# joeylitalien/drmlt-mitsuba

Measured on AMD Instinct MI355X. Metric: mutations/sec (accepted+rejected), higher is better.
Workload: dtype f32

## Files before the change

drmlt-mitsuba_amd/csrc/device_path.h:

```cpp
#pragma once
#include "device_bsdf.h"
#include "device_math.h"
#include "device_sampler.h"
#include "device_types.h"

struct Hit {
    int prim;
    float t, u, v;
};

typedef uint32_t u32x4_t __attribute__((ext_vector_type(4)));
template <class T> DEV T load_global16(const T *p) {
    static_assert(sizeof(T) % 16 == 0, "records are read in 16-byte words");
    typedef const u32x4_t __attribute__((address_space(1))) *GQ;
    const GQ q = (GQ) (uintptr_t) p;
    union { T v; u32x4_t w[sizeof(T) / 16]; } u;
#pragma unroll
    for (unsigned i = 0; i < sizeof(T) / 16u; ++i) u.w[i] = q[i];
    return u.v;
}
DEV f3 smooth_record_sum(const DParams &P, float index_bits, float u, float v) {
    typedef float f32x3_t __attribute__((ext_vector_type(3)));
    typedef const char __attribute__((address_space(1))) *GB;
    typedef const f32x3_t __attribute__((address_space(1))) *GQ;
// ... 422 lines not shown
        load(p, A);
        for (int i = 0; i < n; i += 2, p += 2) {
            PINF(A);
            load(p + 1, B);
            test_flat<TRI>(A, o, d, tmin, best_t, best_uv, best_ks);
            if (i + 1 < n) {
                PINF(B);
                load(p + 2, A);
                test_flat<TRI>(B, o, d, tmin, best_t, best_uv, best_ks);
            }
        }
    }
#undef PINF
    Hit h{-1, best_t, best_uv.x, best_uv.y};
    if (best_ks >= 0) {
        if (best_ks & BOX_FACE_FLAG) {
            const uint32_t hc = (uint32_t) best_ks & 0xffffu;
            const float uu = (hc & 2u) ? h.v : h.u, vv = (hc & 2u) ? h.u : h.v;
            h.u = (hc & 4u) ? 1.f - uu : uu;
            h.v = (hc & 8u) ? 1.f - vv : vv;
            best_ks = (int) (((hc >> 4) & 3u) | ((hc >> 6) << 8));
        }
        h.prim = best_ks >> 8;
        if ((best_ks & 0xff) == PRIM_QUAD2) {
            const bool second = h.v > h.u;
            const float uu = second ? h.u : h.u - h.v, vv = second ? h.v - h.u : h.v;
            h.prim += second ? 1 : 0;
            h.u = uu; h.v = vv;
        }
    }
    return h;
}

template <int FEAT = 15> DEV Hit trace(const DParams &P, f3 o, f3 d, float tmin, float tmax, bool any_hit) {
    if ((FEAT & 8) && P.use_bvh) return trace_bvh(P, o, d, tmin, tmax, any_hit);
    if (P.prims_flat) {
        Hit h = P.has_plain_tri ? trace_flat<true>(P, o, d, tmin, tmax) : trace_flat<false>(P, o, d, tmin, tmax);
        if (FEAT & 4)
            for (int i = P.n_flat; i < P.n_prims; ++i) {
                ScalarPrimPtr sp = (ScalarPrimPtr) (uintptr_t) P.prims;
                DPrim G;
#pragma unroll
                for (int k = 0; k < 12; ++k) G.m[k] = sp[i].m[k];
                const int ks = sp[i].kind_shade;
                G.type = PRIM_SPHERE; G.shade = ks >> 8;
                intersect_prim<4>(G, G.shade, o, d, tmin, h);
            }
        return h;
    }
    return trace_brute<FEAT>(P, o, d, tmin, tmax);
}

struct GlobalTables {
    const DShade *sh; const DBsdf *bs; const DEmitter *em;
    DEV DShade shade(int i) const { return load_global16(sh + i); }
    DEV DBsdf bsdf(int i) const { return load_global16(bs + i); }
    DEV DEmitter emitter(int i) const { return load_global16(em + i); }
    DEV float emitter_cdf_lo(int i) const { return load_global_f32(&em[i].cdf_lo); }
    DEV DShade emitter_shade(int, const DEmitter &E) const { return shade(E.prim); }
};
struct LdsTables {
    uint32_t shade_off, bsdf_off, emit_off;
    DEV DShade shade(int i) const {
        const float4 *q = reinterpret_cast<const float4 *>(&lds_x[shade_off + (uint32_t) i * 16u]);
        const float4 a = q[0], b = q[1], c = q[2], d = q[3];
        DShade s;
// ... 622 lines not shown
```

drmlt-mitsuba_amd/csrc/drmlt_capi.cpp:

```cpp
#include "../../include/drmlt_abi.h"
#include "device_types.h"
#include "drmlt_ctx.h"
#include "scene_prep.h"
#include "bdpt_layers.h"

#include <hip/hip_runtime.h>

#include <algorithm>
#include <chrono>
#include <cmath>
#include <cstdarg>
#include <cstdio>
#include <cstdlib>
#include <cstring>
#include <string>
#include <vector>

void launch_bootstrap(const DParams &P, uint32_t n, float *lum_out, hipStream_t st);
void launch_init_chains(const DParams &P, const uint32_t *seed_index, const float *seed_lum, hipStream_t st);
void launch_mutate(const ChainPlan &plan, const DParams &P, uint32_t n_mut, uint32_t mut_base, hipStream_t st);
void launch_eval_paths(const DParams &P, const float *u, uint32_t n, uint32_t dim, float *out8, hipStream_t st);
void launch_bootstrap_mmlt(const DParams &P, uint32_t n, float *lum_out, size_t lds, hipStream_t st);
void launch_init_chains_mmlt(const DParams &P, const uint32_t *seed_index, const float *seed_lum, size_t lds, hipStream_t st);
void launch_mutate_mmlt(const ChainPlan &plan, const DParams &P, uint32_t n_mut, uint32_t mut_base, hipStream_t st);
// ... 583 lines not shown
    }
    launch_develop(ctx->P.film, d_direct.as<float>(), ctx->P.importance, (float) factor, n, d_out.as<float>(), ctx->stream);
    HIP_TRY(ctx, hipGetLastError());
    HIP_TRY(ctx, hipMemcpyAsync(out_rgb, d_out.p, (size_t) n * sizeof(float), hipMemcpyDeviceToHost, ctx->stream));
    HIP_TRY(ctx, hipStreamSynchronize(ctx->stream));
    return DRMLT_OK;
}

int drmlt_stats_get(drmlt_ctx *ctx, drmlt_stats *o) {
    if (!ctx || !o) return DRMLT_E_INVALID;
    HIP_TRY(ctx, hipSetDevice(ctx->device));
    unsigned long long v[32];
    HIP_TRY(ctx, hipMemcpyAsync(v, ctx->d_stats.p, sizeof v, hipMemcpyDeviceToHost, ctx->stream));
    HIP_TRY(ctx, hipStreamSynchronize(ctx->stream));
    if ((ctx->P.debug & 128) && ctx->cfg.technique == DRMLT_TECH_BDPT)
        fprintf(stderr, "[drmlt stamps] bdpt cycles per wave, summed: walks %llu pair loop %llu whole chain loop %llu | evaluations %llu | stages (all evaluations) %llu, weights + splats %llu, counters + commit %llu\n",
                v[16], v[17], v[18], v[19], v[20], v[21], v[22]);
    else if ((ctx->P.debug & 128) && ctx->P.kernel_variant == 5)
        fprintf(stderr, "[drmlt v5] cycles per wave, summed: bookkeeping %llu step %llu trace %llu | outer iterations %llu, bookkeeping branches %llu (%.1f chains each), "
                        "stepping chains per iteration %.1f, trace phases %llu starting with %.1f lanes, refills %llu\n",
                v[16], v[18], v[17], v[19], v[23], v[23] ? (double) v[24] / v[23] : 0.0, v[19] ? (double) v[25] / v[19] : 0.0, v[20], v[20] ? (double) v[21] / v[20] : 0.0, v[22]);
    else if (ctx->P.debug & 128)
        fprintf(stderr, "[drmlt stamps] cycles: mh %llu trace %llu step %llu | iterations %llu mh-branches %llu tracing-lanes %llu\n",
                v[16], v[17], v[18], v[19], v[20], v[21]),
        fprintf(stderr, "[drmlt stamps] mh sections: decide+splat %llu commit %llu start %llu fill %llu\n", v[22], v[23], v[24], v[25]),
        fprintf(stderr, "[drmlt stamps] iterations by chains tracing (of 32): 0: %llu, 1-4: %llu, 5-8: %llu, 9-16: %llu, 17-24: %llu, 25-32: %llu\n", v[26], v[27], v[28], v[29], v[30], v[31]);
    if (ctx->knobs.verbose && v[12])
        fprintf(stderr, "[drmlt bvh] wave iterations: inner %llu (%.1f lanes each), leaf %llu (%.1f lanes each)\n", v[12], (double) v[10] / (double) v[12], v[13],
                v[13] ? (double) v[11] / (double) v[13] : 0.0);
    if (ctx->knobs.verbose && ctx->P.kernel_variant == 4)
        fprintf(stderr, "[drmlt v4] waves through the orbital rule body: %llu\n", v[14]),
        fprintf(stderr, "[drmlt v4] waves through a one-light build: %llu\n", v[15]);
    if (ctx->knobs.verbose && ctx->P.kernel_variant == 4 && !(ctx->P.debug & 128))
        fprintf(stderr, "[drmlt v4] waves through k_mutate_w2: %llu\n", v[16]);
    if ((ctx->P.debug & 1024) && v[20] && ctx->P.kernel_variant != 5)
        fprintf(stderr, "[drmlt bvh] lanes at slice start, of 64: tracing %.1f, chain waiting for its partner %.1f, chain parked for bookkeeping %.1f, helper idle %.1f, flush %.1f (%llu slices)\n",
                (double) v[21] / v[20], (double) v[22] / v[20], (double) v[23] / v[20], (double) v[24] / v[20], (double) v[25] / v[20], v[20]);
    memset(o, 0, sizeof *o);
    const uint64_t M = ctx->mutations;
    const uint64_t n_large = v[0], acc1_l = v[1], acc1_b = v[2], sec_l = v[3], sec_b = v[4], acc2_l = v[5], acc2_b = v[6], n_rev = v[7];
    if (ctx->cfg.algo == DRMLT_ALGO_PSSMLT) {
        o->overall_base = M;               o->overall_acc = acc1_l + acc1_b;
        o->large_base = n_large;           o->large_acc = acc1_l;
        o->bold_base = M - n_large;        o->bold_acc = acc1_b;
    } else if (!ctx->cfg.use_mixture) {
        o->first_base = M;                 o->first_acc = acc1_l + acc1_b;
        o->large_base = n_large;           o->large_acc = acc1_l;
        o->bold_base = M - n_large;        o->bold_acc = acc1_b;
        o->second_base = sec_l + sec_b;    o->second_acc = acc2_l + acc2_b;
        o->second_large_base = sec_l;      o->second_large_acc = acc2_l;
        o->second_bold_base = sec_b;       o->second_bold_acc = acc2_b;
        o->overall_base = M + sec_l + sec_b;
        o->overall_acc = acc1_l + acc1_b + acc2_l + acc2_b;
    } else {
        o->second_base = sec_b;            o->second_acc = acc2_b;
        o->first_base = M - sec_b;         o->first_acc = acc1_l + acc1_b;
        o->large_base = n_large;           o->large_acc = acc1_l;
        o->bold_base = M - n_large - sec_b; o->bold_acc = acc1_b;
        o->overall_base = M;               o->overall_acc = acc1_l + acc1_b + acc2_b;
    }
    o->mutations = M;
    o->path_evals = M + sec_l + sec_b + n_rev;
    o->rays = v[8];
    o->accepted = acc1_l + acc1_b + acc2_l + acc2_b;
    o->kernel_ms = ctx->kernel_ms;
    o->seed_ms = ctx->seed_ms;
    o->n_chains = ctx->n_chains;
// ... 243 lines not shown
```

drmlt-mitsuba_amd/csrc/kernels.hip:

```cpp
#include <algorithm>
#include <cstdlib>
#include <cstdio>
#include <type_traits>
#include "device_path.h"

#include "kernel_common.h"
#include "launch_plan.h"

__device__ __attribute__((noinline)) DSplat eval_boot_sample(const DParams &P, uint32_t index, uint32_t &nd) {
    Sampler smp;
    smp.key0 = P.key0; smp.key1 = P.key1; smp.chain = P.boot_stream; smp.major = index;
    smp.mode = SM_BOOT; smp.arr = nullptr;
    uint32_t nr;
    return eval_path(P, smp, nr, nd);
}

__global__ void __launch_bounds__(64) k_bootstrap(DParams P, uint32_t n, float *lum_out) {
    uint32_t i = blockIdx.x * blockDim.x + threadIdx.x;
    if (i >= n) return;
    uint32_t nd;
    DSplat s = eval_boot_sample(P, i, nd);
    lum_out[i] = s.lum;
    if (P.boot_weighted) { normalize_splat(s, P); lum_out[(size_t) n + i] = s.lum; }
}
// ... 1058 lines not shown
        helper_has_ray = lower_keeps_u(0u, sr.valid ? 1u : 0u) != 0u;
#else
        const float ox = from_lower(sr.o.x), oy = from_lower(sr.o.y), oz = from_lower(sr.o.z);
        const float dx = from_lower(sr.d.x), dy = from_lower(sr.d.y), dz = from_lower(sr.d.z);
        const float t0 = from_lower(sr.tmin), t1 = from_lower(sr.tmax);
        const float vf = from_lower(sr.valid ? 1.f : 0.f);
        if (helper) {
            ps.o = mk3(ox, oy, oz); ps.d = mk3(dx, dy, dz); ps.tmin = t0; ps.tmax = t1;
            helper_has_ray = vf != 0.f;
        }
#endif
    }
    SECTION_PARAMS(Pe);
    const V4Layout<RULE_ORBITAL> Y = v4_layout<RULE_ORBITAL>(Pe, V4_QCAP);
    if (qn + 32u > Y.L.qcap) W2_FLUSH(Pe, Y.L, qn, lane);
    v4_enqueue(Y.L, qn, live && cum > 0.f, cs.cur.px, cs.cur.py, cs.cur.r * cum, cs.cur.g * cum, cs.cur.b * cum);
    W2_FLUSH(Pe, Y.L, qn, lane);
    if (live) {
        RowSampler smp = Y.smp;
        smp.set_roles(roles, Y.group, sub);
        for (uint32_t k = 0; k < Y.D; ++k) Pe.x[(size_t) k * Pe.n_chains + c] = smp.x(k);
        Pe.cur_lum[c] = cs.cur.lum; Pe.cur_px[c] = cs.cur.px; Pe.cur_py[c] = cs.cur.py;
        Pe.cur_r[c] = cs.cur.r; Pe.cur_g[c] = cs.cur.g; Pe.cur_b[c] = cs.cur.b;
        if (Pe.chain_done) Pe.chain_done[c] = base + cs.it;
    }
    if (Pe.chain_done && !reported && lane == 0) atomicSub(Pe.waves_left, 1u);
    flush_counters(Pe, ct, lane);
    const unsigned long long decided = wave_sum((live && !helper) ? cs.it : 0u);
    if (lane == 0) atomicAdd(Pe.stats + 9, decided);
}
#undef W2_SECTION
#undef W2_FLUSH

#define V5_STACK32_CAP 25
#ifndef V5_ROWS_MEM_WAVES
#define V5_ROWS_MEM_WAVES 3
#endif
#ifndef V5_ROWS_MEM_STACK32_CAP
#define V5_ROWS_MEM_STACK32_CAP 25
#endif
enum { RS_IDLE = 0, RS_BUSY = 1, RS_DONE = 2 };

struct V5Lds {
    uint32_t coin_off, list_off;
    uint32_t q_off;
    uint32_t pool_off;
    uint32_t ring_off;
    uint32_t status_off;
};
DEV V5Lds v5_layout(uint32_t D, uint32_t qcap, bool coin_rows) {
    V5Lds L;
    L.coin_off = D * 64u;
    L.list_off = L.coin_off + (coin_rows ? 4u * 64u : 0u);
    L.q_off = L.list_off + 64u;
    L.pool_off = L.q_off + 5u * qcap;
    L.ring_off = L.pool_off + 8u * V5_SLOTS;
    L.status_off = L.ring_off + V5_SLOTS / 4u;
    return L;
}

template <int FEAT, bool STACK16, bool OVF, bool STAMPS = false, bool LDS_TABLES = false, bool ROWS_MEM = false>
__global__ void __launch_bounds__(CHAIN_BLOCK, ROWS_MEM ? V5_ROWS_MEM_WAVES : 2) k_mutate_v5(DParams P, uint32_t n_mut, uint32_t mut_base) {
    constexpr bool FLAT = (FEAT & 8) == 0;
    typedef typename std::conditional<ROWS_MEM, RowsMem, RowsLds>::type RowsT;
    typedef PoolRowSampler<RowsT> SamplerT;
    constexpr uint32_t QCAP = (FLAT || STACK16) ? V5_QCAP : V5_QCAP_STACK32;
// ... 483 lines not shown
    for (size_t i = (size_t) blockIdx.x * blockDim.x + threadIdx.x; i < n; i += (size_t) gridDim.x * blockDim.x) dst[i] += src[i];
}
void launch_accumulate(float *dst, const float *src, size_t n, hipStream_t st) {
    hipLaunchKernelGGL(k_accumulate, dim3((unsigned) std::min<size_t>((n + 255) / 256, AUX_GRID_CAP)), dim3(256), 0, st, dst, src, n);
}

void launch_bootstrap(const DParams &P, uint32_t n, float *lum_out, hipStream_t st) {
    hipLaunchKernelGGL(k_bootstrap, dim3((n + 63) / 64), dim3(64), 0, st, P, n, lum_out);
}
void launch_init_chains(const DParams &P, const uint32_t *seed_index, const float *seed_lum, hipStream_t st) {
    hipLaunchKernelGGL(k_init_chains, dim3((P.n_chains + 63) / 64), dim3(64), 0, st, P, seed_index, seed_lum);
}
void launch_mutate(const ChainPlan &plan, const DParams &P, uint32_t n_mut, uint32_t mut_base, hipStream_t st) {
    if (plan.verbose && !plan.note.empty()) fprintf(stderr, "%s\n", plan.note.c_str());
#define LAUNCH(...) hipLaunchKernelGGL((__VA_ARGS__), dim3(plan.grid), dim3(CHAIN_BLOCK), plan.lds, st, P, n_mut, mut_base); break
#define LAUNCH_RULE(FEAT, ...) if (orbital) { LAUNCH(k_mutate_v4<FEAT | V4_ORBITAL_BUILD, __VA_ARGS__>); } LAUNCH(k_mutate_v4<FEAT, __VA_ARGS__>)
#define LAUNCH_LIGHT(...) if (one_light) { LAUNCH_RULE(V4_ONE_LIGHT_BUILD, __VA_ARGS__); } LAUNCH_RULE(0, __VA_ARGS__)
    const bool orbital = rule_is_orbital(P), one_light = scene_has_one_light(P);
    switch (plan.build) {
    case Build::PSSMLT: LAUNCH(k_mutate_pssmlt);
    case Build::V5_F0_ROWS: LAUNCH(k_mutate_v5<0, true, false, false, true, true>);   case Build::V5_F1_ROWS: LAUNCH(k_mutate_v5<1, true, false, false, true, true>);
    case Build::V5_F3_ROWS: LAUNCH(k_mutate_v5<3, true, false, false, true, true>);   case Build::V5_F7_ROWS: LAUNCH(k_mutate_v5<7, true, false, false, true, true>);
    case Build::V5_F7_GLOBAL: LAUNCH(k_mutate_v5<7, true, false, false, false>);      case Build::V5_F0_STAMPS: LAUNCH(k_mutate_v5<0, true, false, true, true>);
    case Build::V5_F0: LAUNCH(k_mutate_v5<0, true, false, false, true>);             case Build::V5_F1: LAUNCH(k_mutate_v5<1, true, false, false, true>);
    case Build::V5_F3: LAUNCH(k_mutate_v5<3, true, false, false, true>);             case Build::V5_F7: LAUNCH(k_mutate_v5<7, true, false, false, true>);
    case Build::V5_F8_S32_ROWS: LAUNCH(k_mutate_v5<8, false, true, false, false, true>); case Build::V5_F15_S32_ROWS: LAUNCH(k_mutate_v5<15, false, true, false, false, true>);
    case Build::V5_F8_OVF_ROWS: LAUNCH(k_mutate_v5<8, true, true, false, false, true>);  case Build::V5_F15_OVF_ROWS: LAUNCH(k_mutate_v5<15, true, true, false, false, true>);
    case Build::V5_F8_ROWS: LAUNCH(k_mutate_v5<8, true, false, false, false, true>);     case Build::V5_F15_ROWS: LAUNCH(k_mutate_v5<15, true, false, false, false, true>);
    case Build::V5_F8_S32: LAUNCH(k_mutate_v5<8, false, true>); case Build::V5_F15_S32: LAUNCH(k_mutate_v5<15, false, true>);
    case Build::V5_F8_OVF: LAUNCH(k_mutate_v5<8, true, true>);  case Build::V5_F15_OVF: LAUNCH(k_mutate_v5<15, true, true>);
    case Build::V5_F8_STAMPS: LAUNCH(k_mutate_v5<8, true, false, true>); case Build::V5_F8: LAUNCH(k_mutate_v5<8, true, false>); case Build::V5_F15: LAUNCH(k_mutate_v5<15, true, false>);
    case Build::V4_F0_STAMPS: LAUNCH_LIGHT(true, true);
    case Build::V4_F0:
        if (plan.w2 && orbital && one_light) { LAUNCH(k_mutate_w2); }
        LAUNCH_LIGHT(true, false);
    case Build::V4_F3_STAMPS: LAUNCH(k_mutate_v4<3, true, true>); case Build::V4_F3: LAUNCH_RULE(3, true, false); case Build::V4_F7: LAUNCH_RULE(7, true, false);
    case Build::V4_F15_S32: LAUNCH(k_mutate_v4<15, true, false, false, true>); case Build::V4_F15_OVF: LAUNCH(k_mutate_v4<15, true, false, true, true>);
    case Build::V4_F15: LAUNCH(k_mutate_v4<15, true, false, true>);            case Build::V4_F7_GLOBAL: LAUNCH(k_mutate_v4<7, false, false>);
    case Build::V4_F8_S32_GLOBAL: LAUNCH(k_mutate_v4<8, false, false, false, true>); case Build::V4_F15_S32_GLOBAL: LAUNCH(k_mutate_v4<15, false, false, false, true>);
    case Build::V4_F15_OVF_GLOBAL: LAUNCH(k_mutate_v4<15, false, false, true, true>); case Build::V4_F15_STAMPS_GLOBAL: LAUNCH(k_mutate_v4<15, false, true, true>);
    case Build::V4_F8_GLOBAL: LAUNCH(k_mutate_v4<8, false, false, true>);            case Build::V4_F15_GLOBAL: LAUNCH(k_mutate_v4<15, false, false, true>);
    case Build::V3_F0: LAUNCH(k_mutate_v3<0, true>); case Build::V3_F3: LAUNCH(k_mutate_v3<3, true>); case Build::V3_F7: LAUNCH(k_mutate_v3<7, true>);
    case Build::V3_F15: LAUNCH(k_mutate_v3<15, true>); case Build::V3_F15_GLOBAL: LAUNCH(k_mutate_v3<15, false>);
    default:
        fprintf(stderr, "[drmlt] launch_mutate: build %d is not a technique=path kernel\n", (int) plan.build);
        abort();
    }
#undef LAUNCH_LIGHT
#undef LAUNCH_RULE
#undef LAUNCH
}
void launch_eval_paths(const DParams &P, const float *u, uint32_t n, uint32_t dim, float *out8, hipStream_t st) {
    hipLaunchKernelGGL(k_eval_paths, dim3((n + 63) / 64), dim3(64), 0, st, P, u, n, dim, out8);
}
void launch_render_pt(const DParams &P, uint64_t n_samples, uint32_t stream, float scale, hipStream_t st) {
    hipLaunchKernelGGL(k_render_pt, dim3(16384), dim3(64), 0, st, P, n_samples, stream, scale);
}
void launch_lum_sum(const float *film, const float *importance, uint32_t n_pixels, double *sum, hipStream_t st) {
    hipLaunchKernelGGL(k_lum_sum, dim3(256), dim3(256), 0, st, film, importance, n_pixels, sum);
}
void launch_develop_dev(const float *film, const float *importance, const double *scal, float inv_world, float inv_pixels, int acceptance_map, uint32_t n,
                        float *out, hipStream_t st) {
    hipLaunchKernelGGL(k_develop_dev, dim3(std::min((n + 255) / 256, AUX_GRID_CAP)), dim3(256), 0, st, film, importance, scal, inv_world, inv_pixels, acceptance_map, n, out);
}
void launch_develop(const float *film, const float *direct, const float *importance, float factor, uint32_t n, float *out, hipStream_t st) {
    hipLaunchKernelGGL(k_develop, dim3(std::min((n + 255) / 256, AUX_GRID_CAP)), dim3(256), 0, st, film, direct, importance, factor, n, out);
// ... 2 lines not shown
```

drmlt-mitsuba_amd/csrc/launch_plan.h:

```cpp
#pragma once
#include "../../include/drmlt_abi.h"

#include <algorithm>
#include <cstddef>
#include <cstdint>
#include <cstdio>
#include <cstdlib>
#include <string>

constexpr uint32_t V4_STRIDE = 33u;
constexpr uint32_t V4_QCAP = 160u;
constexpr uint32_t V4_QCAP_BVH = 100u;
constexpr uint32_t V5_QCAP = 96u;
constexpr uint32_t V5_QCAP_STACK32 = 0u;
constexpr uint32_t V5_SLOTS = 128u;

constexpr int bdpt_eval_lds_floats(int max_depth) { return (2 * (2 * max_depth + 1) + 1) * 64; }

inline size_t v3_lds_bytes(size_t D) { return (D + 2 * ((D + 3) & ~(size_t) 3)) * 32 * sizeof(float); }
inline size_t v4_lds_bytes(size_t D, size_t qcap) { return ((D + 2 * ((D + 3) & ~(size_t) 3) + 4) * V4_STRIDE + 32 + 5 * qcap + 3) / 4 * 4 * sizeof(float); }
inline size_t v5_lds_bytes(uint32_t D, uint32_t qcap, bool coin_rows) { return ((size_t) D * 64u + (coin_rows ? 4u * 64u : 0u) + 64u + 5u * qcap + 8u * V5_SLOTS + 2u * (V5_SLOTS / 4u)) * sizeof(float); }
inline size_t mmlt_lds_bytes(int mmlt_S, int mmlt_E, int max_depth) { return ((size_t) mmlt_S + mmlt_E + 1 + 3 * ((size_t) max_depth + 3)) * 64 * sizeof(float); }
inline size_t bdpt_lds_bytes(int mmlt_S, int mmlt_E, int max_depth) { return (((size_t) mmlt_S + mmlt_E) * 64 + (size_t) bdpt_eval_lds_floats(max_depth)) * sizeof(float); }

struct Knobs {
    bool verbose = false;
    int debug = 0;
    int kernel = 0;
    int slice = 1024;
    int bvh_threshold = 48, bvh_max_depth = 64, bvh_leaf = 1;
    bool bvh_stack32 = false;
    bool no_quad_merge = false, no_box_merge = false, no_flat_loop = false, feat_all = false;
    bool tables_lds_off = false;
    int mh_batch = 0, trace_yield = -1, pool_refill = 0, trace_vote = 0;
    int rows_mem = -1;
    bool no_small_tables = false, mmlt_tables_global = false, bdpt_tables_global = false;
    int bdpt_occ = 0;
    size_t bdpt_lds_pad = 0;
    bool no_run_ahead = false;
    bool rule_generic = false;
    bool no_w2 = false;
    bool one_light_generic = false;
    long long ahead_cap = -1;
    bool mmlt_no_sort = false, no_regroup = false, regroup_on_host = false, regroup_check = false;
    int regroup_first = 0;
};

inline Knobs read_knobs() {
    Knobs K;
    const struct { const char *name; bool *on; } flags[] = {
        {"DRMLT_VERBOSE", &K.verbose}, {"DRMLT_BVH_STACK32", &K.bvh_stack32}, {"DRMLT_NO_QUAD_MERGE", &K.no_quad_merge}, {"DRMLT_NO_BOX_MERGE", &K.no_box_merge},
        {"DRMLT_NO_FLAT_LOOP", &K.no_flat_loop}, {"DRMLT_FEAT_ALL", &K.feat_all}, {"DRMLT_NO_SMALL_TABLES", &K.no_small_tables},
        {"DRMLT_MMLT_TABLES_GLOBAL", &K.mmlt_tables_global}, {"DRMLT_BDPT_TABLES_GLOBAL", &K.bdpt_tables_global}, {"DRMLT_NO_RUN_AHEAD", &K.no_run_ahead},
        {"DRMLT_RULE_GENERIC", &K.rule_generic}, {"DRMLT_ONE_LIGHT_GENERIC", &K.one_light_generic}, {"DRMLT_NO_W2", &K.no_w2},
        {"DRMLT_MMLT_NO_SORT", &K.mmlt_no_sort}, {"DRMLT_NO_REGROUP", &K.no_regroup}, {"DRMLT_REGROUP_ON_HOST", &K.regroup_on_host}, {"DRMLT_REGROUP_CHECK", &K.regroup_check}};
    for (const auto &f : flags) *f.on = getenv(f.name) != nullptr;
    int v = 0;
    auto num = [&v](const char *name) { const char *e = getenv(name); if (e) v = atoi(e); return e != nullptr; };
    if (num("DRMLT_DEBUG")) K.debug = v;
    if (num("DRMLT_KERNEL")) K.kernel = v == 3 ? 3 : (v == 5 ? 5 : 4);
    if (num("DRMLT_SLICE")) K.slice = std::max(1, std::min(32768, v));
    if (num("DRMLT_BVH_THRESHOLD")) K.bvh_threshold = v;
    if (num("DRMLT_BVH_MAX_DEPTH")) K.bvh_max_depth = std::min(K.bvh_max_depth, v);
    if (num("DRMLT_BVH_LEAF")) K.bvh_leaf = v;
    if (num("DRMLT_TABLES_LDS")) K.tables_lds_off = v == 0;
    if (num("DRMLT_MH_BATCH")) K.mh_batch = std::max(1, std::min(64, v));
    if (num("DRMLT_TRACE_YIELD")) K.trace_yield = std::max(0, std::min(64, v));
    if (num("DRMLT_POOL_REFILL")) K.pool_refill = std::max(1, std::min(64, v));
    if (num("DRMLT_TRACE_VOTE")) K.trace_vote = std::max(1, std::min(1024, v));
    if (num("DRMLT_ROWS_MEM")) K.rows_mem = v != 0;
    if (num("DRMLT_BDPT_OCC")) K.bdpt_occ = v;
    if (num("DRMLT_BDPT_LDS_PAD")) K.bdpt_lds_pad = (size_t) v;
    if (num("DRMLT_AHEAD_CAP")) K.ahead_cap = std::max(0, v);
    if (num("DRMLT_REGROUP_FIRST")) K.regroup_first = std::max(1, std::min(K.slice, v));
    return K;
}

struct PlanInputs {
    int technique = DRMLT_TECH_PATH, algo = DRMLT_ALGO_DRMLT;
    int work_units = -1, work_units_rule = DRMLT_WORK_UNITS_DEVICE;
    uint64_t budget = 0;
    int features = 0;
    bool use_bvh = false, bvh_stack16 = false;
    bool bvh_overflow = false;
    uint32_t n_shade = 0, n_bsdfs = 0, n_emitters = 0;
    uint64_t scene_bytes = 0;
    int eff_dim = 0, max_depth = 0, mmlt_S = 0, mmlt_E = 0;
    int cus = 256;
};

enum class Build {
    PSSMLT,
    V5_F0_ROWS, V5_F1_ROWS, V5_F3_ROWS, V5_F7_ROWS,
    V5_F7_GLOBAL, V5_F0_STAMPS, V5_F0, V5_F1, V5_F3, V5_F7,
    V5_F8_S32_ROWS, V5_F15_S32_ROWS, V5_F8_OVF_ROWS, V5_F15_OVF_ROWS, V5_F8_ROWS, V5_F15_ROWS,
    V5_F8_S32, V5_F15_S32, V5_F8_OVF, V5_F15_OVF, V5_F8_STAMPS, V5_F8, V5_F15,
    V4_F0_STAMPS, V4_F0, V4_F3_STAMPS, V4_F3, V4_F7, V4_F15_S32, V4_F15_OVF, V4_F15,
    V4_F7_GLOBAL, V4_F8_S32_GLOBAL, V4_F15_S32_GLOBAL, V4_F15_OVF_GLOBAL, V4_F15_STAMPS_GLOBAL, V4_F8_GLOBAL, V4_F15_GLOBAL,
    V3_F0, V3_F3, V3_F7, V3_F15, V3_F15_GLOBAL,
    MMLT_F7_TABLES, MMLT_F15, MMLT_F7,
    BDPT_F15, BDPT_F7_OCC2_TABLES, BDPT_F7_OCC2, BDPT_F7,
    PSSMLT_BDPT_F15, PSSMLT_BDPT_F7_OCC2_TABLES, PSSMLT_BDPT_F7_OCC2, PSSMLT_BDPT_F7,
};

struct ChainPlan {
    Build build = Build::PSSMLT;
    uint32_t chains_per_wave = 64, grid = 0;
    size_t lds = 0;
    size_t aux_lds = 0;
    int kernel_variant = 5, tables_in_lds = 0, small_tables_lds = 0;
    bool rows_mem = false;
    int mh_batch = 0, trace_yield = 0, pool_refill = 0, trace_vote = 0;
    bool w2 = false;
    bool run_ahead = false;
    bool verbose = false;
    std::string note;
};

namespace plan_detail {
inline size_t lds_table_bytes(const PlanInputs &in) { return (size_t) in.n_shade * 64 + (size_t) in.n_bsdfs * 48 + (size_t) in.n_emitters * 32; }
inline size_t small_table_bytes(const PlanInputs &in) { return ((size_t) in.n_bsdfs * 12 + (size_t) in.n_emitters * 24) * sizeof(float); }
inline bool path_mh(const PlanInputs &in) { return in.technique == DRMLT_TECH_PATH && in.algo != DRMLT_ALGO_PSSMLT; }

constexpr size_t CU_LDS_BYTES = 160u * 1024u;
inline bool w2_launch(size_t lds, uint32_t grid, int cus) { return lds * 12u > CU_LDS_BYTES || (uint64_t) grid <= (uint64_t) cus * 4u * 2u; }

struct Family { int variant; bool tables_in_lds, rows_mem; };
inline Family family(const PlanInputs &in, uint32_t n_chains, const Knobs &K) {
    Family f;
    f.tables_in_lds = lds_table_bytes(in) <= 16384 && !K.tables_lds_off;
    f.variant = K.kernel ? K.kernel : 5;
    if (f.variant == 5 && !in.use_bvh && K.kernel != 5 && n_chains < 98304u) f.variant = 4;
    const bool can = f.variant == 5 && (in.use_bvh || f.tables_in_lds) && path_mh(in);
    f.rows_mem = can && (K.rows_mem >= 0 ? K.rows_mem == 1 : (uint64_t) n_chains * 2u >= (uint64_t) in.cus * 4u * 64u * 5u);
    return f;
}
}

inline uint32_t derive_chains(const PlanInputs &in, const Knobs &K) {
    if (in.work_units > 0) return (uint32_t) in.work_units;
    const bool mmlt = in.technique == DRMLT_TECH_MMLT, bdpt = in.technique == DRMLT_TECH_BDPT;
    if (in.work_units_rule == DRMLT_WORK_UNITS_REFERENCE) {
        const uint64_t per_unit = (mmlt || bdpt) ? 100000 : 200000;
        return (uint32_t) std::max<uint64_t>(1, (in.budget + per_unit - 1) / per_unit);
    }
    uint64_t fill = 65536;
    if (in.algo == DRMLT_ALGO_PSSMLT) fill = 65536;
    else if (mmlt) fill = in.budget >= (1ull << 35) ? 1048576 : 262144;
    else if (bdpt) fill = 131072;
    else if (plan_detail::path_mh(in) && !K.kernel) fill = plan_detail::family(in, 196608, K).rows_mem ? 196608 : 131072;
    return (uint32_t) std::min<uint64_t>(fill, std::max<uint64_t>(64, in.budget / 64 / 64 * 64));
}

inline ChainPlan plan_chains(const PlanInputs &in, uint32_t n_chains, const Knobs &K) {
    using namespace plan_detail;
    ChainPlan p;
    const Family f = family(in, n_chains, K);
    const bool mmlt = in.technique == DRMLT_TECH_MMLT, bdpt = in.technique == DRMLT_TECH_BDPT, pssmlt = in.algo == DRMLT_ALGO_PSSMLT;
// ... 33 lines not shown
        if (pssmlt)
            p.build = p.build == Build::BDPT_F15 ? Build::PSSMLT_BDPT_F15 : p.build == Build::BDPT_F7_OCC2_TABLES ? Build::PSSMLT_BDPT_F7_OCC2_TABLES
                    : p.build == Build::BDPT_F7_OCC2 ? Build::PSSMLT_BDPT_F7_OCC2 : Build::PSSMLT_BDPT_F7;
    } else if (pssmlt) {
        waves(64);
        p.lds = D * 64 * sizeof(float);
        p.build = Build::PSSMLT;
    } else if (f.variant == 5) {
        waves(64);
        const bool flat = (F & 8) == 0, diffuse = F == 8;
        p.lds = v5_lds_bytes(f.rows_mem ? 0u : (uint32_t) D, (flat || s16) ? V5_QCAP : V5_QCAP_STACK32, flat || s16);
        if (flat) p.lds += tables;
        else if (p.small_tables_lds) p.lds += small_table_bytes(in);
        snprintf(note, sizeof note, "[drmlt] k_mutate_v5: %zu B of LDS per wave%s%s", p.lds, flat ? "" : " (+ the traversal stack)",
                 f.rows_mem ? "; proposal rows in device memory, three waves per SIMD" : "");
        if (flat && f.rows_mem) p.build = F == 0 ? Build::V5_F0_ROWS : F == 1 ? Build::V5_F1_ROWS : (F & ~3) == 0 ? Build::V5_F3_ROWS : Build::V5_F7_ROWS;
        else if (flat && !f.tables_in_lds) p.build = Build::V5_F7_GLOBAL;
        else if (flat) p.build = F == 0 ? (stamps ? Build::V5_F0_STAMPS : Build::V5_F0) : F == 1 ? Build::V5_F1 : (F & ~3) == 0 ? Build::V5_F3 : Build::V5_F7;
        else if (f.rows_mem) p.build = !s16 ? (diffuse ? Build::V5_F8_S32_ROWS : Build::V5_F15_S32_ROWS) : ovf ? (diffuse ? Build::V5_F8_OVF_ROWS : Build::V5_F15_OVF_ROWS)
                                                                  : (diffuse ? Build::V5_F8_ROWS : Build::V5_F15_ROWS);
        else p.build = !s16 ? (diffuse ? Build::V5_F8_S32 : Build::V5_F15_S32) : ovf ? (diffuse ? Build::V5_F8_OVF : Build::V5_F15_OVF)
                                                        : diffuse ? (stamps ? Build::V5_F8_STAMPS : Build::V5_F8) : Build::V5_F15;
    } else if (f.variant == 4) {
        waves(32);
        p.lds = v4_lds_bytes(D, (F & 8) ? V4_QCAP_BVH : V4_QCAP) + tables;
        snprintf(note, sizeof note, "[drmlt] k_mutate_v4: %zu B of LDS per wave", p.lds);
        if (f.tables_in_lds)
            p.build = F == 0 ? (stamps ? Build::V4_F0_STAMPS : Build::V4_F0) : (F & ~3) == 0 ? (stamps ? Build::V4_F3_STAMPS : Build::V4_F3)
                    : (F & 8) == 0 ? Build::V4_F7 : !s16 ? Build::V4_F15_S32 : ovf ? Build::V4_F15_OVF : Build::V4_F15;
        else
            p.build = (F & 8) == 0 ? Build::V4_F7_GLOBAL : !s16 ? (F == 8 ? Build::V4_F8_S32_GLOBAL : Build::V4_F15_S32_GLOBAL) : ovf ? Build::V4_F15_OVF_GLOBAL
                    : stamps ? Build::V4_F15_STAMPS_GLOBAL : F == 8 ? Build::V4_F8_GLOBAL : Build::V4_F15_GLOBAL;
        p.w2 = p.build == Build::V4_F0 && !K.no_w2 && w2_launch(p.lds, p.grid, in.cus);
    } else {
        waves(32);
        p.lds = v3_lds_bytes(D) + tables;
        snprintf(note, sizeof note, "[drmlt] k_mutate_v3: %zu B of LDS per wave", p.lds);
        p.build = !f.tables_in_lds ? Build::V3_F15_GLOBAL : F == 0 ? Build::V3_F0 : (F & ~3) == 0 ? Build::V3_F3 : (F & 8) == 0 ? Build::V3_F7 : Build::V3_F15;
    }
    p.note = note;
    return p;
}
```

drmlt-mitsuba_amd/csrc/scene_prep.h:

```cpp
#pragma once
#include "../../include/drmlt_abi.h"
#include "box_merge.h"
#include "bvh_build.h"
#include "device_types.h"
#include "launch_plan.h"

#include <algorithm>
#include <array>
#include <cmath>
#include <cstdio>
#include <cstring>
#include <limits>
#include <string>
#include <vector>

struct PreparedScene {
    std::vector<DPrim> prims;
    std::vector<DShade> shade;
    std::vector<DBsdf> bsdfs;
    std::vector<DEmitter> emitters;
    std::vector<DBvh4Node> bvh;
    std::vector<DPrimFlat> flat;
    std::vector<DPrimBox> boxes;
    std::vector<DSmooth> normals;
// ... 455 lines not shown
        P.eff_dim = P.mmlt_S + P.mmlt_E + 1;
    }
    if (cfg.technique == DRMLT_TECH_BDPT) {
        const int rr = cfg.max_depth + 1 - (cfg.rr_depth > 0 ? cfg.rr_depth : 0);
        P.mmlt_S = 2 * (cfg.max_depth + 1) + (rr > 0 ? rr : 0); P.mmlt_S += P.mmlt_S & 1;
        P.mmlt_E = 2 * cfg.max_depth + (rr > 1 ? rr - 1 : 0); P.mmlt_E += P.mmlt_E & 1;
        P.mmlt_dmax = (cfg.max_depth + 2) * (2 + (cfg.rr_depth < cfg.max_depth ? 1 : 0)); P.mmlt_dmax += P.mmlt_dmax & 1;
        P.bd_Dd = cfg.no_direct_sampling ? 0 : 2 * (2 * cfg.max_depth - 1);
        P.max_dim = 2 * P.mmlt_dmax + P.bd_Dd;
        P.eff_dim = P.mmlt_S + P.mmlt_E + P.bd_Dd;
    }

    P.debug = K.debug | (K.rule_generic ? DBG_RULE_GENERIC : 0) | (K.one_light_generic ? DBG_ONE_LIGHT_GENERIC : 0);
    if (!out.emitters.empty()) { P.light = out.emitters[0]; P.light_shade = out.shade[(size_t) out.emitters[0].prim]; }
    for (const DBsdf &b : out.bsdfs) P.features |= b.type == DRMLT_BSDF_ROUGHCONDUCTOR ? 1 : ((b.type == DRMLT_BSDF_DIELECTRIC || b.type == DRMLT_BSDF_CONDUCTOR) ? 2 : 0);
    for (const DPrim &g : out.prims) if (g.type == PRIM_SPHERE) P.features |= 4;
    if (!out.normals.empty()) P.features |= 4;
    P.env_emitter = -1;
    for (int i = 0; i < scene.n_emitters; ++i) {
        if (scene.emitters[i].type == DRMLT_EMITTER_POINT) P.features |= 4;
        if (scene.emitters[i].type == DRMLT_EMITTER_CONSTANT) P.features |= 4, P.env_emitter = i;
    }
    if (P.use_bvh) P.features |= 8;
    if (K.feat_all) P.features = 15;

    PlanInputs &in = out.plan;
    in.technique = cfg.technique; in.algo = cfg.algo;
    in.work_units = cfg.work_units; in.work_units_rule = cfg.work_units_rule;
    in.budget = (uint64_t) cam.width * cam.height * (uint64_t) cfg.sample_count;
    in.features = P.features; in.use_bvh = P.use_bvh != 0; in.bvh_stack16 = P.bvh_stack16 != 0; in.bvh_overflow = out.ovf_entries > 0;
    in.n_shade = (uint32_t) P.n_shade; in.n_bsdfs = (uint32_t) P.n_bsdfs; in.n_emitters = (uint32_t) P.n_emitters;
    in.scene_bytes = P.use_bvh ? (uint64_t) P.n_bvh_nodes * sizeof(DBvh4Node) + out.prims.size() * sizeof(DPrim) : 0;
    in.eff_dim = P.eff_dim; in.max_depth = cfg.max_depth; in.mmlt_S = P.mmlt_S; in.mmlt_E = P.mmlt_E;
    return "";
}
```

Measured before the change: 3.048 billion.

## Add w2 mutate kernel holding tiny-scene ray records in registers

Adds k_mutate_w2h, a variant of the w2 orbital one-light kernel that loads up to three merged box records and one flat record into registers once per wave and traces rays against them directly. This replaces the per-ray global loads of the flat scene records. The plan selects it when the scene fits those limits and has no plain triangles, and an env knob can turn it off. The cost is higher register pressure, a duplicated kernel body, and a new trace path that must match the existing box/quad hit decoding.

```diff
diff --git a/drmlt-mitsuba_amd/csrc/device_path.h b/drmlt-mitsuba_amd/csrc/device_path.h
--- a/drmlt-mitsuba_amd/csrc/device_path.h
+++ b/drmlt-mitsuba_amd/csrc/device_path.h
@@ -478,6 +478,38 @@
     return h;
 }
 
+struct HeldScene {
+    BoxRec box[3];
+    FlatRec flat;
+};
+DEV Hit trace_held(const HeldScene &S, uint32_t n_box, uint32_t n_flat, f3 o, f3 d, float tmin, float tmax) {
+    float best_t = tmax;
+    float2v best_uv = {0.f, 0.f};
+    int best_ks = -1;
+    if (n_box > 0u) test_box(S.box[0], o, d, tmin, best_t, best_uv, best_ks);
+    if (n_box > 1u) test_box(S.box[1], o, d, tmin, best_t, best_uv, best_ks);
+    if (n_box > 2u) test_box(S.box[2], o, d, tmin, best_t, best_uv, best_ks);
+    if (n_flat > 0u) test_flat<false>(S.flat, o, d, tmin, best_t, best_uv, best_ks);
+    Hit h{-1, best_t, best_uv.x, best_uv.y};
+    if (best_ks >= 0) {
+        if (best_ks & BOX_FACE_FLAG) {
+            const uint32_t hc = (uint32_t) best_ks & 0xffffu;
+            const float uu = (hc & 2u) ? h.v : h.u, vv = (hc & 2u) ? h.u : h.v;
+            h.u = (hc & 4u) ? 1.f - uu : uu;
+            h.v = (hc & 8u) ? 1.f - vv : vv;
+            best_ks = (int) (((hc >> 4) & 3u) | ((hc >> 6) << 8));
+        }
+        h.prim = best_ks >> 8;
+        if ((best_ks & 0xff) == PRIM_QUAD2) {
+            const bool second = h.v > h.u;
+            const float uu = second ? h.u : h.u - h.v, vv = second ? h.v - h.u : h.v;
+            h.prim += second ? 1 : 0;
+            h.u = uu; h.v = vv;
+        }
+    }
+    return h;
+}
+
 template <int FEAT = 15> DEV Hit trace(const DParams &P, f3 o, f3 d, float tmin, float tmax, bool any_hit) {
     if ((FEAT & 8) && P.use_bvh) return trace_bvh(P, o, d, tmin, tmax, any_hit);
     if (P.prims_flat) {
diff --git a/drmlt-mitsuba_amd/csrc/drmlt_capi.cpp b/drmlt-mitsuba_amd/csrc/drmlt_capi.cpp
--- a/drmlt-mitsuba_amd/csrc/drmlt_capi.cpp
+++ b/drmlt-mitsuba_amd/csrc/drmlt_capi.cpp
@@ -639,7 +639,8 @@
         fprintf(stderr, "[drmlt v4] waves through the orbital rule body: %llu\n", v[14]),
         fprintf(stderr, "[drmlt v4] waves through a one-light build: %llu\n", v[15]);
     if (ctx->knobs.verbose && ctx->P.kernel_variant == 4 && !(ctx->P.debug & 128))
-        fprintf(stderr, "[drmlt v4] waves through k_mutate_w2: %llu\n", v[16]);
+        fprintf(stderr, "[drmlt v4] waves through k_mutate_w2: %llu\n", v[16]),
+        fprintf(stderr, "[drmlt v4] waves with the ray records held in registers: %llu\n", v[17]);
     if ((ctx->P.debug & 1024) && v[20] && ctx->P.kernel_variant != 5)
         fprintf(stderr, "[drmlt bvh] lanes at slice start, of 64: tracing %.1f, chain waiting for its partner %.1f, chain parked for bookkeeping %.1f, helper idle %.1f, flush %.1f (%llu slices)\n",
                 (double) v[21] / v[20], (double) v[22] / v[20], (double) v[23] / v[20], (double) v[24] / v[20], (double) v[25] / v[20], v[20]);
diff --git a/drmlt-mitsuba_amd/csrc/kernels.hip b/drmlt-mitsuba_amd/csrc/kernels.hip
--- a/drmlt-mitsuba_amd/csrc/kernels.hip
+++ b/drmlt-mitsuba_amd/csrc/kernels.hip
@@ -1114,6 +1114,278 @@
 #undef W2_SECTION
 #undef W2_FLUSH
 
+struct W2HeldScene {
+    HeldScene S;
+    uint32_t counts;
+};
+template <class Rec> DEV void w2_hold_rows(Rec &G, const float *c, const float *rz, bool have) {
+    float v[12];
+#pragma unroll
+    for (int k = 0; k < 12; ++k) v[k] = 0.f;
+    if (have) {
+#pragma unroll
+        for (int k = 0; k < 8; ++k) v[k] = c[k];
+#pragma unroll
+        for (int k = 0; k < 4; ++k) v[8 + k] = rz[k];
+    }
+#pragma unroll
+    for (int k = 0; k < 12; ++k) hold_v(v[k]);
+    G.cx = float2v{v[0], v[1]}; G.cy = float2v{v[2], v[3]}; G.cz = float2v{v[4], v[5]}; G.cw = float2v{v[6], v[7]};
+    G.z0 = v[8]; G.z1 = v[9]; G.z2 = v[10]; G.z3 = v[11];
+}
+DEV W2HeldScene w2_held_scene(const DParams &P) {
+    W2HeldScene H;
+    const uint32_t n_box = (uint32_t) min(max(P.n_box, 0), 3), n_flat = (uint32_t) min(max(P.n_flat_rec, 0), 1);
+#pragma unroll
+    for (uint32_t i = 0; i < 3u; ++i) {
+        BoxRec &G = H.S.box[i];
+        const DPrimBox *q = P.prims_box + i;
+        w2_hold_rows(G, q->c, q->rz, i < n_box);
+        uint32_t f0 = 0u, f1 = 0u, f2 = 0u;
+        if (i < n_box) { f0 = q->fw[0]; f1 = q->fw[1]; f2 = q->fw[2]; }
+        hold_v(f0); hold_v(f1); hold_v(f2);
+        G.f0 = f0; G.f1 = f1; G.f2 = f2;
+    }
+    FlatRec &F = H.S.flat;
+    w2_hold_rows(F, P.prims_flat->c, P.prims_flat->rz, n_flat > 0u);
+    int ks = -1;
+    if (n_flat > 0u) ks = P.prims_flat->kind_shade;
+    hold_v(ks);
+    F.ks = ks;
+    H.counts = n_box | (n_flat << 8);
+    hold_v(H.counts);
+    return H;
+}
+
+__global__ void __launch_bounds__(CHAIN_BLOCK, 2) k_mutate_w2h(DParams P, uint32_t n_mut, uint32_t mut_base) {
+    typedef RowSamplerT<RULE_ORBITAL> RowSampler;
+    if (threadIdx.x == 0) { atomicAdd(P.stats + 14, 1ull); atomicAdd(P.stats + 15, 1ull); atomicAdd(P.stats + 16, 1ull); atomicAdd(P.stats + 17, 1ull); }
+    const uint32_t lane = threadIdx.x;
+    const uint32_t sub = lane & 31u;
+    const bool helper = lane >= 32u;
+    const uint32_t c = blockIdx.x * 32u + sub;
+    const bool live = !helper && c < P.n_chains;
+    const uint32_t cc = c < P.n_chains ? c : P.n_chains - 1;
+    const uint32_t S = V4_STRIDE;
+    int smp_mode = SM_STAGE1;
+    uint32_t roles;
+    uint32_t qn = 0u;
+    ChainState cs;
+    float cum = 0.f;
+    Counters ct = {0u, 0u, 0u, 0u, 0u};
+    PathState ps;
+    bool helper_has_ray = false;
+    Hit h{-1, 0.f, 0.f, 0.f};
+    int batch;
+    uint32_t base = 0u, target = 0u, limit = 0u;
+    bool reported = false;
+    W2Held held = w2_held(P);
+    w2_hold(held);
+    const W2HeldScene scene = w2_held_scene(P);
+    uint32_t imp_lo = (uint32_t) (uintptr_t) P.importance, imp_hi = (uint32_t) ((uintptr_t) P.importance >> 32);
+    uint32_t done_lo = (uint32_t) (uintptr_t) P.chain_done, done_hi = (uint32_t) ((uintptr_t) P.chain_done >> 32);
+    uint32_t left_lo = (uint32_t) (uintptr_t) P.waves_left, left_hi = (uint32_t) ((uintptr_t) P.waves_left >> 32);
+    uint32_t key0_v = P.key0, key1_v = P.key1, chain_off_v = P.chain_offset, timid_v = (uint32_t) P.timid_after_large;
+    hold_v(imp_lo); hold_v(imp_hi); hold_v(done_lo); hold_v(done_hi); hold_v(left_lo); hold_v(left_hi);
+    hold_v(key0_v); hold_v(key1_v); hold_v(chain_off_v); hold_v(timid_v);
+    {
+        const V4Layout<RULE_ORBITAL> Y = v4_layout<RULE_ORBITAL>(P, V4_QCAP);
+        roles = RowSampler::first_roles(Y.group, sub);
+        if (!helper) {
+            for (uint32_t k = 0; k < Y.D; ++k) lds_x[k * S + sub] = unwrap01(P.x[(size_t) k * P.n_chains + cc]);
+            for (uint32_t k = Y.D; k < Y.D4; ++k) lds_x[k * S + sub] = 0.f;
+        }
+        cs.cur.lum = P.cur_lum[cc]; cs.cur.px = P.cur_px[cc]; cs.cur.py = P.cur_py[cc];
+        cs.cur.r = P.cur_r[cc]; cs.cur.g = P.cur_g[cc]; cs.cur.b = P.cur_b[cc];
+        cs.y = cs.cur; cs.z = cs.cur;
+        cs.a1 = 0.f; cs.coin_acc1 = cs.coin_acc2 = cs.coin_mix = 0.f;
+        cs.it = 0u; cs.nd1 = cs.nd2 = 0u; cs.stage = -1; cs.large = false;
+        path_init(P, ps);
+        base = (P.chain_done && live) ? P.chain_done[cc] : mut_base;
+        target = P.chain_done ? n_mut : mut_base + n_mut;
+        limit = P.chain_done ? P.run_limit : target;
+        ps.phase = (live && base < limit) ? PH_DONE : PH_IDLE;
+        ps.o = mk3(0.f, 0.f, 0.f); ps.d = mk3(0.f, 0.f, 1.f); ps.tmin = 0.f; ps.tmax = 0.f;
+        batch = P.mh_batch > 32 ? 32 : P.mh_batch;
+        stage_tables(P, Y.LT, lane);
+        if (!helper) {
+            const u4 coins = philox4x32_10(P.key0, P.key1, 0u, base, P.chain_offset + blockIdx.x * 32u + sub, TAG_COIN);
+            float *dst = &lds_x[Y.L.coin_off + sub];
+            dst[0] = u32_to_unit(coins.x); dst[S] = u32_to_unit(coins.y); dst[2u * S] = u32_to_unit(coins.z); dst[3u * S] = u32_to_unit(coins.w);
+        }
+    }
+
+    for (;;) {
+        const bool parked = ps.phase == PH_DONE;
+        const unsigned long long pmask = __ballot(parked);
+        const unsigned long long rmask = __ballot(ps.phase != PH_DONE && ps.phase != PH_IDLE);
+        if (!pmask && !rmask) break;
+        if (pmask && (__popcll(pmask) >= batch || !rmask)) {
+            DParams Pm{};
+            Pm.importance = uniform_ptr<const float>(imp_lo, imp_hi); Pm.width = (int) wave_uniform((uint32_t) held.width); Pm.height = (int) wave_uniform((uint32_t) held.height);
+            Pm.chain_done = uniform_ptr<uint32_t>(done_lo, done_hi); Pm.waves_left = uniform_ptr<uint32_t>(left_lo, left_hi);
+            Pm.key0 = wave_uniform(key0_v); Pm.key1 = wave_uniform(key1_v); Pm.chain_offset = wave_uniform(chain_off_v);
+            Pm.eff_dim = (int) wave_uniform((uint32_t) held.eff_dim); Pm.timid_after_large = (int) wave_uniform(timid_v);
+            Pm.use_mixture = 0; Pm.acceptance_map = 0; Pm.type = 2;
+            const W2Held &C = held;
+            const V4Lds L{C.coin_off, C.list_off, C.q_off, C.qcap};
+            RowSampler smp = w2_sampler(Pm.key0, Pm.key1);
+            smp.set_roles(roles, C.group, sub); smp.mode = smp_mode;
+            const uint32_t D4 = ((uint32_t) Pm.eff_dim + 3u) & ~3u, nb1 = D4 / 4u;
+            int *const lds_list = reinterpret_cast<int *>(&lds_x[L.list_off]);
+            __builtin_amdgcn_s_setprio(2);
+            if (qn + 64u > wave_uniform(L.qcap)) { SECTION_PARAMS(Pf); w2_flush(Pf, L, qn, lane); }
+            int commit = 0, kind = 0;
+            bool wantA = false, wantB = false;
+            float eAx = 0.f, eAy = 0.f, eAr = 0.f, eAg = 0.f, eAb = 0.f;
+            float eBx = 0.f, eBy = 0.f, eBr = 0.f, eBg = 0.f, eBb = 0.f;
+            if (parked) {
+                const MhDigest o = mh_decide<RULE_ORBITAL>(Pm, cs, smp, ps, ct);
+                if (o.decided) {
+                    cum += o.w.w0;
+                    const bool a1st = o.acc1, a2nd = o.acc2, adopt = a1st || a2nd;
+                    const DSplat sb = select_splat(a2nd, cs.y, cs.z);
+                    const float wb = a2nd ? o.w.w1 : o.w.w2;
+                    wantB = !a1st && wb > 0.f;
+                    eBx = sb.px; eBy = sb.py; eBr = sb.r * wb; eBg = sb.g * wb; eBb = sb.b * wb;
+                    const DSplat sa = select_splat(adopt, cs.cur, cs.y);
+                    const float wa = adopt ? cum : o.w.w1;
+                    wantA = wa > 0.f;
+                    eAx = sa.px; eAy = sa.py; eAr = sa.r * wa; eAg = sa.g * wa; eAb = sa.b * wa;
+                    if (adopt) {
+                        cum = a1st ? o.w.w1 : o.w.w2;
+                        cs.cur = select_splat(a1st, cs.y, cs.z);
+                    }
+                    commit = mh_commit_mode(o);
+                }
+                kind = cs.stage < 0 ? 4 : 2;
+            }
+            kind = mh_resolve_kind(Pm, kind, live, base + cs.it, target, limit, reported, lane);
+            v4_enqueue(L, qn, wantA, eAx, eAy, eAr, eAg, eAb);
+            v4_enqueue(L, qn, wantB, eBx, eBy, eBr, eBg, eBb);
+
+            smp.adopt(commit);
+            roles = smp.roles();
+
+            if (parked && kind == 1) {
+                const float *cn = &lds_x[L.coin_off + sub];
+                cs.large = cn[0] < C.p_large;
+                cs.coin_acc1 = cn[S]; cs.coin_acc2 = cn[2u * S]; cs.coin_mix = cn[3u * S];
+                cs.stage = 0;
+                cs.nd1 = cs.nd2 = 0u;
+            }
+
+            RowSampler smg = w2_sampler(Pm.key0, Pm.key1);
+            const uint32_t chain_base_g = Pm.chain_offset + blockIdx.x * 32u;
+            const uint32_t maj_mine = base + cs.it;
+            const unsigned info = roles | (cs.large ? 1u : 0u);
+            const uint32_t f1mask = (uint32_t) __ballot(kind == 1);
+            if (f1mask) {
+                if (kind == 1) lds_list[__builtin_amdgcn_mbcnt_lo(f1mask, 0u)] = (int) sub;
+                const uint32_t n = (uint32_t) __popc(f1mask), total = n * (nb1 + 1u);
+                const float rcp_n = 1.f / (float) n;
+                for (uint32_t fb = 0u; fb < total; fb += 64u) {
+                    const uint32_t i = fb + lane;
+                    const bool valid = i < total;
+                    const uint32_t ii = valid ? i : 0u;
+                    const uint32_t b = (uint32_t) (((float) ii + 0.5f) * rcp_n), j = ii - b * n;
+                    const uint32_t cj = (uint32_t) lds_list[j];
+                    const uint32_t mj = (uint32_t) __shfl((int) maj_mine, (int) cj, 64);
+                    const unsigned inf = (unsigned) __shfl((int) info, (int) cj, 64);
+                    smg.set_roles(inf, C.group, cj);
+                    const bool coin = b >= nb1;
+                    if (valid) {
+                        const u4 r = philox4x32_10(Pm.key0, Pm.key1, coin ? 0u : b, coin ? mj + 1u : mj, chain_base_g + cj, coin ? TAG_COIN : TAG_S1);
+                        const Unit4 u{{u32_to_unit(r.x), u32_to_unit(r.y), u32_to_unit(r.z), u32_to_unit(r.w)}};
+                        if (!coin) row_fill_first_drawn(smg, b, u, (inf & 1u) != 0u);
+                        else {
+                            float *dst = &lds_x[L.coin_off + cj];
+                            dst[0] = u.v[0]; dst[S] = u.v[1]; dst[2u * S] = u.v[2]; dst[3u * S] = u.v[3];
+                        }
+                    }
+                }
+            }
+            const uint32_t f2mask = (uint32_t) __ballot(kind == 2);
+            if (f2mask) {
+                if (kind == 2) lds_list[__builtin_amdgcn_mbcnt_lo(f2mask, 0u)] = (int) sub;
+                const uint32_t nb2 = Pm.timid_after_large ? D4 / 4u : (D4 / 2u + 3u) / 4u;
+                const uint32_t n = (uint32_t) __popc(f2mask), total = n * nb2;
+                const float rcp_n = 1.f / (float) n;
+                for (uint32_t fb = 0u; fb < total; fb += 64u) {
+                    const uint32_t i = fb + lane;
+                    const bool valid = i < total;
+                    const uint32_t ii = valid ? i : 0u;
+                    const uint32_t b = (uint32_t) (((float) ii + 0.5f) * rcp_n), j = ii - b * n;
+                    const uint32_t cj = (uint32_t) lds_list[j];
+                    const uint32_t mj = (uint32_t) __shfl((int) maj_mine, (int) cj, 64);
+                    const unsigned inf = (unsigned) __shfl((int) info, (int) cj, 64);
+                    smg.set_roles(inf, C.group, cj);
+                    if (valid) smg.fill_second(b, D4, mj, chain_base_g + cj, (inf & 1u) != 0u);
+                }
+            }
+
+            if (parked) {
+                if (kind == 0) ps.phase = PH_IDLE;
+                else {
+                    DParams Vb{};
+                    Vb.exclude_direct = C.exclude_direct; Vb.width = C.width; Vb.height = C.height;
+                    Vb.tan_half_fov = C.tan_half_fov; Vb.inv_aspect = C.inv_aspect; Vb.near_clip = C.near_clip; Vb.far_clip = C.far_clip;
+#pragma unroll
+                    for (int q = 0; q < 12; ++q) Vb.cam[q] = C.cam[q];
+                    smp_mode = smp.mode = cs.stage == 0 ? SM_STAGE1 : SM_STAGE2;
+                    path_init(Vb, ps);
+                    const float v0 = smp.next(0u), v1 = smp.next(1u);
+                    path_begin(Vb, ps, v0, v1);
+                }
+            }
+        }
+        const bool tracing = helper ? helper_has_ray : ps.phase == PH_CLOSEST;
+        __builtin_amdgcn_s_setprio(0);
+        if (__ballot(tracing)) {
+            const uint32_t counts = wave_uniform(scene.counts);
+            h = trace_held(scene.S, counts & 0xffu, counts >> 8, ps.o, ps.d, ps.tmin, ps.tmax);
+        }
+        __builtin_amdgcn_s_setprio(3);
+        const unsigned occluded = from_upper_u((helper_has_ray && h.prim >= 0) ? 1u : 0u);
+        helper_has_ray = false;
+        ShadowRay sr;
+        asm volatile("" : "=v"(sr.d.x), "=v"(sr.d.y), "=v"(sr.d.z), "=v"(sr.tmin), "=v"(sr.tmax));
+        sr.o = ps.o; sr.valid = false;
+        {
+            const W2Held &Cs = held;
+            if (!helper && ps.phase != PH_DONE && ps.phase != PH_IDLE) {
+                RowSampler sms = w2_sampler(0u, 0u);
+                sms.set_roles(roles, Cs.group, sub); sms.mode = smp_mode;
+                DParams Vs{};
+                Vs.eff_dim = Cs.eff_dim; Vs.rr_depth = Cs.rr_depth; Vs.max_depth = Cs.max_depth;
+                const LdsTables LT{Cs.shade_off, Cs.bsdf_off, 0u};
+                path_step_diffuse<RowSampler, HeldLightTables, false>(Vs, HeldLightTables{LT, Cs.light, Cs.light_shade}, ps, sms, h, occluded == 0u, sr);
+            }
+        }
+        ps.o.x = lower_keeps(ps.o.x, sr.o.x); ps.o.y = lower_keeps(ps.o.y, sr.o.y); ps.o.z = lower_keeps(ps.o.z, sr.o.z);
+        ps.d.x = lower_keeps(ps.d.x, sr.d.x); ps.d.y = lower_keeps(ps.d.y, sr.d.y); ps.d.z = lower_keeps(ps.d.z, sr.d.z);
+        ps.tmin = lower_keeps(ps.tmin, sr.tmin); ps.tmax = lower_keeps(ps.tmax, sr.tmax);
+        helper_has_ray = lower_keeps_u(0u, sr.valid ? 1u : 0u) != 0u;
+    }
+    SECTION_PARAMS(Pe);
+    const V4Layout<RULE_ORBITAL> Y = v4_layout<RULE_ORBITAL>(Pe, V4_QCAP);
+    if (qn + 32u > Y.L.qcap) w2_flush(Pe, Y.L, qn, lane);
+    v4_enqueue(Y.L, qn, live && cum > 0.f, cs.cur.px, cs.cur.py, cs.cur.r * cum, cs.cur.g * cum, cs.cur.b * cum);
+    w2_flush(Pe, Y.L, qn, lane);
+    if (live) {
+        RowSampler smp = Y.smp;
+        smp.set_roles(roles, Y.group, sub);
+        for (uint32_t k = 0; k < Y.D; ++k) Pe.x[(size_t) k * Pe.n_chains + c] = smp.x(k);
+        Pe.cur_lum[c] = cs.cur.lum; Pe.cur_px[c] = cs.cur.px; Pe.cur_py[c] = cs.cur.py;
+        Pe.cur_r[c] = cs.cur.r; Pe.cur_g[c] = cs.cur.g; Pe.cur_b[c] = cs.cur.b;
+        if (Pe.chain_done) Pe.chain_done[c] = base + cs.it;
+    }
+    if (Pe.chain_done && !reported && lane == 0) atomicSub(Pe.waves_left, 1u);
+    flush_counters(Pe, ct, lane);
+    const unsigned long long decided = wave_sum((live && !helper) ? cs.it : 0u);
+    if (lane == 0) atomicAdd(Pe.stats + 9, decided);
+}
+
 #define V5_STACK32_CAP 25
 #ifndef V5_ROWS_MEM_WAVES
 #define V5_ROWS_MEM_WAVES 3
@@ -1663,6 +1935,7 @@
     case Build::V5_F8_STAMPS: LAUNCH(k_mutate_v5<8, true, false, true>); case Build::V5_F8: LAUNCH(k_mutate_v5<8, true, false>); case Build::V5_F15: LAUNCH(k_mutate_v5<15, true, false>);
     case Build::V4_F0_STAMPS: LAUNCH_LIGHT(true, true);
     case Build::V4_F0:
+        if (plan.w2_held && orbital && one_light) { LAUNCH(k_mutate_w2h); }
         if (plan.w2 && orbital && one_light) { LAUNCH(k_mutate_w2); }
         LAUNCH_LIGHT(true, false);
     case Build::V4_F3_STAMPS: LAUNCH(k_mutate_v4<3, true, true>); case Build::V4_F3: LAUNCH_RULE(3, true, false); case Build::V4_F7: LAUNCH_RULE(7, true, false);
diff --git a/drmlt-mitsuba_amd/csrc/launch_plan.h b/drmlt-mitsuba_amd/csrc/launch_plan.h
--- a/drmlt-mitsuba_amd/csrc/launch_plan.h
+++ b/drmlt-mitsuba_amd/csrc/launch_plan.h
@@ -40,6 +40,7 @@
     bool no_run_ahead = false;
     bool rule_generic = false;
     bool no_w2 = false;
+    bool no_w2_held = false;
     bool one_light_generic = false;
     long long ahead_cap = -1;
     bool mmlt_no_sort = false, no_regroup = false, regroup_on_host = false, regroup_check = false;
@@ -52,7 +53,7 @@
         {"DRMLT_VERBOSE", &K.verbose}, {"DRMLT_BVH_STACK32", &K.bvh_stack32}, {"DRMLT_NO_QUAD_MERGE", &K.no_quad_merge}, {"DRMLT_NO_BOX_MERGE", &K.no_box_merge},
         {"DRMLT_NO_FLAT_LOOP", &K.no_flat_loop}, {"DRMLT_FEAT_ALL", &K.feat_all}, {"DRMLT_NO_SMALL_TABLES", &K.no_small_tables},
         {"DRMLT_MMLT_TABLES_GLOBAL", &K.mmlt_tables_global}, {"DRMLT_BDPT_TABLES_GLOBAL", &K.bdpt_tables_global}, {"DRMLT_NO_RUN_AHEAD", &K.no_run_ahead},
-        {"DRMLT_RULE_GENERIC", &K.rule_generic}, {"DRMLT_ONE_LIGHT_GENERIC", &K.one_light_generic}, {"DRMLT_NO_W2", &K.no_w2},
+        {"DRMLT_RULE_GENERIC", &K.rule_generic}, {"DRMLT_ONE_LIGHT_GENERIC", &K.one_light_generic}, {"DRMLT_NO_W2", &K.no_w2}, {"DRMLT_NO_W2_HELD", &K.no_w2_held},
         {"DRMLT_MMLT_NO_SORT", &K.mmlt_no_sort}, {"DRMLT_NO_REGROUP", &K.no_regroup}, {"DRMLT_REGROUP_ON_HOST", &K.regroup_on_host}, {"DRMLT_REGROUP_CHECK", &K.regroup_check}};
     for (const auto &f : flags) *f.on = getenv(f.name) != nullptr;
     int v = 0;
@@ -87,6 +88,8 @@
     uint64_t scene_bytes = 0;
     int eff_dim = 0, max_depth = 0, mmlt_S = 0, mmlt_E = 0;
     int cus = 256;
+    int n_box = 0, n_flat_rec = 0;
+    bool has_plain_tri = false;
 };
 
 enum class Build {
@@ -112,6 +115,7 @@
     bool rows_mem = false;
     int mh_batch = 0, trace_yield = 0, pool_refill = 0, trace_vote = 0;
     bool w2 = false;
+    bool w2_held = false;
     bool run_ahead = false;
     bool verbose = false;
     std::string note;
@@ -124,6 +128,7 @@
 
 constexpr size_t CU_LDS_BYTES = 160u * 1024u;
 inline bool w2_launch(size_t lds, uint32_t grid, int cus) { return lds * 12u > CU_LDS_BYTES || (uint64_t) grid <= (uint64_t) cus * 4u * 2u; }
+inline bool w2_held_launch(int n_box, int n_flat_rec, bool has_plain_tri) { return n_box >= 1 && n_box <= 3 && n_flat_rec >= 0 && n_flat_rec <= 1 && !has_plain_tri; }
 
 struct Family { int variant; bool tables_in_lds, rows_mem; };
 inline Family family(const PlanInputs &in, uint32_t n_chains, const Knobs &K) {
@@ -223,6 +228,7 @@
             p.build = (F & 8) == 0 ? Build::V4_F7_GLOBAL : !s16 ? (F == 8 ? Build::V4_F8_S32_GLOBAL : Build::V4_F15_S32_GLOBAL) : ovf ? Build::V4_F15_OVF_GLOBAL
                     : stamps ? Build::V4_F15_STAMPS_GLOBAL : F == 8 ? Build::V4_F8_GLOBAL : Build::V4_F15_GLOBAL;
         p.w2 = p.build == Build::V4_F0 && !K.no_w2 && w2_launch(p.lds, p.grid, in.cus);
+        p.w2_held = p.w2 && !K.no_w2_held && w2_held_launch(in.n_box, in.n_flat_rec, in.has_plain_tri);
     } else {
         waves(32);
         p.lds = v3_lds_bytes(D) + tables;
diff --git a/drmlt-mitsuba_amd/csrc/scene_prep.h b/drmlt-mitsuba_amd/csrc/scene_prep.h
--- a/drmlt-mitsuba_amd/csrc/scene_prep.h
+++ b/drmlt-mitsuba_amd/csrc/scene_prep.h
@@ -511,5 +511,6 @@
     in.n_shade = (uint32_t) P.n_shade; in.n_bsdfs = (uint32_t) P.n_bsdfs; in.n_emitters = (uint32_t) P.n_emitters;
     in.scene_bytes = P.use_bvh ? (uint64_t) P.n_bvh_nodes * sizeof(DBvh4Node) + out.prims.size() * sizeof(DPrim) : 0;
     in.eff_dim = P.eff_dim; in.max_depth = cfg.max_depth; in.mmlt_S = P.mmlt_S; in.mmlt_E = P.mmlt_E;
+    in.n_box = P.n_box; in.n_flat_rec = P.n_flat_rec; in.has_plain_tri = P.has_plain_tri != 0;
     return "";
 }
```

Result: faster. 3.275 billion (median of 6 runs) (+7.4%).
